# tomtor/HDL-deflate

Hardware: AMD Instinct MI355X
Metric: compress_input_throughput (CWINDOW=32, MATCH10=True, static tree) (higher is better)
Workload: dtype u8; 1 GPU; BASELINE configs[1]: 1048576 x 2048 B blocks, families 1-4 (test_deflate.py:38-66), distinct blocks, HBM-resident; cwindow=32, maxmatch=10, blocks_per_gpu=1048576, block_bytes=2048

## Files before the change

### __graft_entry__.py

```python
import os
import subprocess
import sys

REPO = os.path.dirname(os.path.abspath(__file__))
if REPO not in sys.path:
    sys.path.insert(0, REPO)


def build():
    subprocess.check_call(["bash", os.path.join(REPO, "hdl_deflate_amd", "csrc", "build.sh")])
    subprocess.check_call(["bash", os.path.join(REPO, "hdl_deflate_amd", "csrc", "build.sh"), "forced"])
    subprocess.check_call(["bash", os.path.join(REPO, "hdl_deflate_amd", "csrc", "build.sh"), "keys"])
    subprocess.check_call(["bash", os.path.join(REPO, "hdl_deflate_amd", "csrc", "build.sh"), "alllive"])
    subprocess.check_call(["make", "-s", "-C", os.path.join(REPO, "oracle"), "all"])
    import hdl_deflate_amd
    from hdl_deflate_amd import _lib
    L = _lib.load()
    hdr = open(os.path.join(REPO, "include", "hdlz.h")).read()
    import re
    want = int(re.search(r"#define\s+HDLZ_VERSION\s+(0x[0-9a-fA-F]+)", hdr).group(1), 16)
    assert L.hdlz_version() == want, (hex(L.hdlz_version()), hex(want))
    for name in _lib.EXPORTS:
        assert hasattr(L, name), name
    return None


def smoke():
    import zlib
    import torch
    import hdl_deflate_amd
    from hdl_deflate_amd.data import make_blocks
    from oracle import oracle as O
    assert torch.cuda.is_available(), "smoke() needs cuda:0"
    torch.cuda.set_device(0)
    eng = hdl_deflate_amd.Engine()
    d = make_blocks(64, 2048, "cuda", seed=1)
    out, ol, st = eng.compress_batch(d, cwindow=32, maxmatch=10)
    back, bl, bs = eng.inflate_batch(out, out_pitch=2048)
    torch.cuda.synchronize()
    assert int((st != 0).sum()) == 0 and int((bs != 0).sum()) == 0
    assert torch.equal(back, d)
    h, ho, hl = d.cpu().numpy(), out.cpu().numpy(), ol.cpu().numpy()
    for b in range(64):
        blk = h[b].tobytes()
        z = ho[b, :hl[b]].tobytes()
        rc, ref = O.compress(blk, 32, 10)
        assert rc == 0 and z == ref, "block %d differs from the oracle" % b
        assert zlib.decompress(z) == blk
    blk0 = h[0].tobytes()
    ses = eng.compress_session()
    for k in range(0, len(blk0), 300):
        ses.write(blk0[k:k + 300])
        assert ses.step() == 0
    assert ses.step(final=True) == 0 and ses.done and ses.output(0, ses.out_len) == O.compress(blk0, 32, 10)[1]
    st1, z = eng.compress_bytes(b"Hello World! " * 3)
    assert st1 == 0 and z.hex() == "789cf348cdc9c95708cf2fca4951544070101c10475101000c2f0d18"
    print("smoke OK: 64 x 2 KiB blocks bit-identical to the oracle, zlib round trip, ratio %.3f" %
          (hl.sum() / (64 * 2048.0)))
    return None


if __name__ == "__main__":
    build()
    if len(sys.argv) > 1 and sys.argv[1] == "smoke":
        smoke()
```

### hdl_deflate_amd/csrc/hdlz_compress.hip

```cpp
#include <hip/hip_runtime.h>
#include <stdint.h>
#include "hdlz_device.h"
#include "hdlz_compress_common.h"

namespace hdlz {

#ifndef HDLZ_HP_SEARCH
#define HDLZ_HP_SEARCH 1
#define HDLZ_HP_EXTEND 0
#define HDLZ_HP_REST 0
#endif
#ifdef HDLZ_TILE_TIMING
#define TT_DECL() uint32_t tacc[13] = {0, 0, 0, 0, 0, 0, 0, 0, 0, 0, 0, 0, 0}, tlast = (uint32_t)__builtin_readcyclecounter(); \
        const uint32_t tt_c0 = tlast, tt_r0 = (uint32_t)__builtin_amdgcn_s_memrealtime()
#define TT(k) do { const uint32_t t_ = (uint32_t)__builtin_readcyclecounter(); tacc[k] += t_ - tlast; tlast = t_; } while (0)
#define TT_TILE() tacc[12] += 1u
#else
#define TT_DECL() do {} while (0)
#define TT(k) do {} while (0)
#define TT_TILE() do {} while (0)
#endif

__device__ __forceinline__ void store_words(uint32_t* __restrict__ dst, const uint32_t* lsrc, uint32_t words, uint32_t lane) {
    typedef uint32_t v4 __attribute__((ext_vector_type(4)));
// ... 59 lines not shown
        const uint8_t* t = reinterpret_cast<const uint8_t*>(FIXED_LUT.e) + 16u * lane;
        lds_dma16(t, lut_base);
        lds_dma16(t + 1024u, lut_base + 1024u);
    };

#if defined(HDLZ_STRIDE_PLAIN) || defined(HDLZ_TILE_TIMING)
    constexpr bool MOVING_COLUMN = false;
#else
    constexpr bool MOVING_COLUMN = BITS;
#endif
    [[maybe_unused]] uint64_t row0 = 0;
    [[maybe_unused]] uint32_t col = blockIdx.x;
    auto next_block = [&](uint64_t& blk) {
        if constexpr (MOVING_COLUMN) {
            row0 += gridDim.x;
            col = col + 1u == gridDim.x ? 0u : col + 1u;
            blk = row0 + col;
        } else blk += gridDim.x;
    };
    TT_DECL();
    for (uint64_t blk = blockIdx.x; blk < a.nblocks; next_block(blk)) {
        const uint8_t* src;
        uint32_t n;
        const uint32_t bst = block_params(blk, src, n);
        if (bst != HDLZ_OK) {
            if (lane == 0) {
                a.out_len[blk] = 0; a.status[blk] = bst;
                if constexpr (ENDBITS) a.end_bits[blk] = 0;
            }
            continue;
        }
        uint32_t* __restrict__ outw = reinterpret_cast<uint32_t*>(a.out + blk * a.out_pitch);
        const uint32_t mis = (uint32_t)(reinterpret_cast<uintptr_t>(src) & 3u);
        const bool aligned16 = (reinterpret_cast<uintptr_t>(src) & 15u) == 0;

        uint32_t gw = 0;
        uint32_t base_bits = HEADER_BITS;
        uint32_t carry_word = HEADER_WORD;
        uint32_t skip_in = 0;
        uint32_t ad_a = 0, ad_w = 0;
        uint32_t wm = (n - min(lane * (uint32_t)RUN, n)) % ADLER_MOD;

        for (uint32_t t0 = 0; t0 < n; t0 += TILE) {
            if (blk == blockIdx.x) TT(10); else TT(0);
            HDLZ_MARK("stage");
            const uint32_t nfull = min((n - t0) >> 4, NCHUNK);
            wave_lds_order();
            lds.in[lane] = t0 != 0 ? lds.in[(TILE / 4) + lane] : 0u;
            asm volatile("s_waitcnt lgkmcnt(0)" ::: "memory");
            request_tile(src + t0, nfull);
            {
                const uint32_t part = (nfull < NCHUNK && ((n - t0) & 15u) != 0u) ? 1u : 0u;
                for (uint32_t c = nfull + part + lane; c < NCHUNK; c += 64) *reinterpret_cast<uint4*>(lin8 + HALO + c * 16u) = make_uint4(0, 0, 0, 0);
                if (part) {
                    if (lane == 0u) *reinterpret_cast<uint4*>(lin8 + HALO + nfull * 16u) = load_chunk16(src, t0 + nfull * 16u, n, aligned16, mis);
                }
            }
            if constexpr (!HASH && !BITS) zero_bit_buffer(lout, lane, carry_word);
            asm volatile("s_waitcnt vmcnt(0)" ::: "memory");
            wave_lds_order();

            const uint32_t run_dw = (HALO / 4) + lane * (RUN / 4);
            const uint32_t p_run = t0 + lane * RUN;
            const uint32_t nrem = n - min(p_run, n);
            uint32_t best[RUN], tok[RUN], code[RUN];
            [[maybe_unused]] uint32_t oww[12];
            [[maybe_unused]] bool any = true;
            [[maybe_unused]] uint32_t planes[7];
            if constexpr (BITS) {
                load_own(lds.in, run_dw, oww);
                asm volatile("s_waitcnt lgkmcnt(0)" ::: "memory");
                wave_lds_order();
            }
            TT(1);
            if constexpr (!HASH) __builtin_amdgcn_s_setprio(0);
            else __builtin_amdgcn_s_setprio(HDLZ_HP_SEARCH);
            HDLZ_MARK("search");
            if constexpr (HASH) {
                match_search_hash<NCH>(lds.in, hl, lane, (uint32_t)a.cwindow, best);
                zero_bit_buffer(lout, lane, carry_word);
            }
#ifndef HDLZ_SEARCH_KEYS
            else if constexpr (BITS)
                any = match_search_bits<true>(oww[0], oww[1], oww[2], oww[3], oww[4], oww[5], oww[6], oww[7], planes, lds.neq + lane);
#endif
            else match_search<NCH, ONE_TILE && NCH == 1>(lds.in, run_dw, best);
            {
                TT(2);
                HDLZ_MARK("adler");
                uint32_t ow[12];
                if constexpr (BITS) {
#pragma unroll
                    for (int k = 0; k < 12; k++) ow[k] = oww[k];
                } else load_own(lds.in, run_dw, ow);
                {
                    uint32_t sa, sc;
                    adler_run(ow, sa, sc);
                    ad_a += sa;
                    ad_w = (ad_w + __umul24(wm, sa) + (4u * ADLER_MOD - sc)) % ADLER_MOD;
                    wm = wm >= (uint32_t)(TILE % ADLER_MOD) ? wm - (uint32_t)(TILE % ADLER_MOD) : wm + (ADLER_MOD - (uint32_t)(TILE % ADLER_MOD));
                    if (((t0 >> 11) & 0x3FFFFu) == 0x3FFFFu) ad_a %= ADLER_MOD;
                    asm volatile("" : "+v"(ad_a), "+v"(ad_w), "+v"(wm));
                }
                TT(3);
                if constexpr (!HASH) __builtin_amdgcn_s_setprio(1);
                else __builtin_amdgcn_s_setprio(HDLZ_HP_EXTEND);
                HDLZ_MARK("extend");
                if constexpr (BITS) {
                    if (any) {
                        search_result_bytes(planes, best);
                        wave_lds_order();
                        make_tokens_bits<FULLWIN>(lds.neq, lane, ow, best, cw4, kmax, 4u * min(p_run, 32u * NCH), nrem, tok, (int32_t)(n - t0));
                    } else {
                        literal_tokens(ow, tok);
                        asm volatile("s_waitcnt lgkmcnt(0)" ::: "memory");
                        wave_lds_order();
                    }
                } else
                make_tokens<NCH, FULLWIN, true>(lds.in, HALO + lane * RUN, ow, best, cw4, kmax, 4u * min(p_run, 32u * NCH), nrem, tok, (int32_t)(n - t0));
            }
            pin(tok);
            PHASE_FENCE();
            TT(4);
            if constexpr (BITS) {
                HDLZ_MARK("zero");
                wave_lds_order();
                request_lut();
                zero_bit_buffer(lout, lane, carry_word);
            }
            if constexpr (HASH) __builtin_amdgcn_s_setprio(HDLZ_HP_REST);
            HDLZ_MARK("parse");
            uint32_t myskip = 0;
            if (!BITS || any) {
                const uint64_t P = run_transfer(tok);
                TT(5);
                HDLZ_MARK("chain");
                myskip = chain_skips(P, lane, skip_in);
            }
            pin(tok); asm volatile("" : "+v"(myskip));
            PHASE_FENCE();
            TT(6);
            HDLZ_MARK("codes");
            if constexpr (BITS) {
                asm volatile("s_waitcnt vmcnt(0)" ::: "memory");
                wave_lds_order();
            }
            uint32_t lane_bits = token_codes<NCH, false>(lut8, tok, myskip, 0u, code);
            pin(code);
            PHASE_FENCE();
            TT(7);
            HDLZ_MARK("scan");
            uint32_t incl = wave_scan_incl(lane_bits);
            const uint32_t tile_bits_all = (uint32_t)__builtin_amdgcn_readlane((int)incl, 63);
            pin(code); asm volatile("" : "+v"(incl), "+v"(lane_bits));
            PHASE_FENCE();
            TT(8);
            HDLZ_MARK("scatter");
            scatter_codes(out8, code, base_bits + incl - lane_bits);
            TT(9);
            HDLZ_MARK("flush");
            wave_lds_order();
            TT(10);

            const bool last = ONE_TILE || (t0 + TILE >= n);
            if (!last) {
                const uint32_t end_bits = base_bits + tile_bits_all;
                const uint32_t full = end_bits >> 5;
                store_words(outw + gw, lout, full, lane);
                carry_word = lout[full];
                gw += full;
                base_bits = end_bits & 31u;
            } else {
                const uint32_t ninv = t0 + TILE - n;
                const uint32_t end_bits = base_bits + tile_bits_all - PAD_BITS * ninv;
                if (lane < 4u) wipe_behind(lout, end_bits, lane);
                uint32_t s1, s2;
                adler_finish(wave_sum(ad_a % ADLER_MOD), wave_sum(ad_w), n, s1, s2);
                const uint32_t nbytes = block_nbytes(end_bits);
                wave_lds_order();
                if (lane == 0) put_adler(out8, nbytes, s1, s2);
                wave_lds_order();
                const uint32_t total = nbytes + 4u;
                const uint32_t words = (total + 3u) >> 2;
                store_words(outw + gw, lout, words, lane);
                if (lane == 0) {
                    a.out_len[blk] = gw * 4u + total;
                    a.status[blk] = HDLZ_OK;
                    if constexpr (ENDBITS) a.end_bits[blk] = 32ull * gw + end_bits;
                }
            }
            TT(11);
            TT_TILE();
        }
    }
#ifdef HDLZ_TILE_TIMING
// ... 62 lines not shown
```

### hdl_deflate_amd/csrc/hdlz_compress_common.h

```cpp
#pragma once
#include <hip/hip_runtime.h>
#include <stddef.h>
#include <stdint.h>
#include "hdlz_device.h"
#include "hdlz_adler.h"

namespace hdlz {

#ifndef HDLZ_W1
#define HDLZ_W1 5
#endif

#ifndef HDLZ_EXT_GROUP
#define HDLZ_EXT_GROUP 4
#endif
#ifndef HDLZ_CODE_GROUP
#define HDLZ_CODE_GROUP 4
#endif
constexpr int RUN = 32;
constexpr int TILE = 64 * RUN;
constexpr int HALO = 256;
constexpr int LOOKAHEAD = 16;
constexpr int IN_BYTES = HALO + TILE + LOOKAHEAD;
constexpr int OUT_WORDS = 592;
constexpr int LUT_LIT = 256;
constexpr int LUT_MATCH = 256;
constexpr uint32_t LUT_MATCH_BYTE = 4u * LUT_LIT;
constexpr int LUT_LEN = 16;
constexpr uint32_t LUT_LEN_BYTE = 4u * (LUT_LIT + LUT_MATCH);
constexpr uint32_t NB_SHIFT = 27;
constexpr uint32_t CODE_MASK = (1u << NB_SHIFT) - 1u;

struct __attribute__((aligned(16))) WaveLds {
    uint32_t in[IN_BYTES / 4];
    uint32_t out[OUT_WORDS];
    uint32_t lut[LUT_LIT + LUT_MATCH + LUT_LEN];
};

constexpr uint32_t GATHER_SPAN = 4u * (0x3FFu + 3u);
static_assert(sizeof(WaveLds) >= GATHER_SPAN, "make_tokens: masked gather inside the LDS block");

constexpr int NEQ_ROWS = 32;
constexpr int NEQ_WORDS = NEQ_ROWS * 64;
constexpr int FIXED_LUT_WORDS = LUT_LIT + LUT_MATCH;
constexpr bool search_bits() {
#ifdef HDLZ_SEARCH_KEYS
    return false;
#else
    return true;
#endif
}
struct __attribute__((aligned(16))) WaveLdsBits {
    union {
        uint32_t in[IN_BYTES / 4];
        uint32_t neq[NEQ_WORDS];
        struct {
            uint32_t out[OUT_WORDS];
            uint32_t gap[NEQ_WORDS - OUT_WORDS - FIXED_LUT_WORDS];
            uint32_t lut[FIXED_LUT_WORDS];
        };
    };
};
static_assert((0x7C << 6) + 4 * 63 + 4 <= 4 * NEQ_WORDS && ((0xFF & 0x7C) << 6) == 4 * 64 * 31, "every read of the extension inside NEQ; none -> row 31");
static_assert(((4 * 32) & 0x7C) == 0 && (31 * 64 + 63) < NEQ_WORDS, "d = 32 aliases row 0; the search's last row ends inside NEQ");
static_assert(sizeof(WaveLdsBits) == 8192 && 4 * NEQ_WORDS >= IN_BYTES, "20 waves per CU; the staged tile inside the block");
static_assert(offsetof(WaveLdsBits, lut) >= 4 * OUT_WORDS && offsetof(WaveLdsBits, lut) % 16 == 0 && 4 * FIXED_LUT_WORDS == 2 * 64 * 16,
              "zero_bit_buffer leaves the LUT alone; the LUT is two 16-byte LDS-DMA requests per lane");

struct __attribute__((aligned(16))) WaveLdsNoOut {
    uint32_t in[IN_BYTES / 4];
    uint32_t lut[LUT_LIT + LUT_MATCH + LUT_LEN];
};

#define PHASE_FENCE() __builtin_amdgcn_sched_barrier(0)
#define HDLZ_MARK(name) do { PHASE_FENCE(); asm volatile("; @@PHASE " name ::: "memory"); PHASE_FENCE(); } while (0)
template <int N>
__device__ __forceinline__ void pin(uint32_t (&a)[N]) {
#pragma unroll
    for (int i = 0; i < N; i++) asm volatile("" : "+v"(a[i]));
}
template <int B, int E, int N>
__device__ __forceinline__ void pin_range(uint32_t (&a)[N]) {
#pragma unroll
    for (int i = B; i < E; i++) asm volatile("" : "+v"(a[i]));
}

__device__ __forceinline__ uint32_t alignbyte(uint32_t hi, uint32_t lo, uint32_t sh) {
    return __builtin_amdgcn_alignbyte(hi, lo, sh);
}
__device__ __forceinline__ uint32_t umin3(uint32_t a, uint32_t b, uint32_t c) {
    uint32_t t = a < b ? a : b;
    return t < c ? t : c;
}
__device__ __forceinline__ uint32_t ffbl(uint32_t x) { return (uint32_t)(__builtin_ffs((int)x) - 1); }

template <int J>
__device__ __forceinline__ uint32_t key3(const uint32_t* d, uint32_t tag) {
    constexpr int w = J >> 2, sh = J & 3;
    if constexpr (sh == 0) return (d[w] << 8) | tag;
    else if constexpr (sh == 1) return (d[w] & 0xFFFFFF00u) | tag;
    else return (alignbyte(d[w + 1], d[w], sh - 1) & 0xFFFFFF00u) | tag;
}

__host__ __device__ constexpr uint32_t literal_entry(uint32_t b) {
    const bool big = b >= 144u;
    const uint32_t v = big ? (0x100u + b) : (0x30u + b);
    const uint32_t nb = big ? 9u : 8u;
    return (__builtin_bitreverse32(v) >> (32u - nb)) | (nb << NB_SHIFT);
}
__host__ __device__ constexpr uint32_t dist_entry(uint32_t d) {
    const uint32_t dd = d - 1u;
    uint32_t c = dd, eb = 0, extra = 0;
    if (dd >= 4u) {
        const uint32_t hb = 31u - (uint32_t)__builtin_clz(dd);
        eb = hb - 1u;
        c = 2u * hb + ((dd >> eb) & 1u);
        extra = dd & ((1u << eb) - 1u);
    }
    const uint32_t dcode = __builtin_bitreverse32(c) >> 27;
    return ((dcode | (extra << 5)) << 7) | ((12u + eb) << NB_SHIFT);
}
__host__ __device__ constexpr uint32_t length_code(uint32_t m) { return __builtin_bitreverse32(m - 2u) >> 25; }
static_assert(literal_entry(0) == (0x0Cu | 8u << NB_SHIFT), "literal 0: 8 bits, 00110000 reversed");
static_assert(literal_entry(143) == (0xFDu | 8u << NB_SHIFT), "literal 143: 8 bits, 10111111 reversed");
static_assert(literal_entry(144) == (0x13u | 9u << NB_SHIFT), "literal 144: 9 bits, 110010000 reversed");
static_assert(literal_entry(255) == (0x1FFu | 9u << NB_SHIFT), "literal 255: 9 bits, all ones");
static_assert(length_code(3) == 0x40u && length_code(10) == 0x08u, "lengths 3 / 10: symbols 257 / 264 = 7-bit codes 0000001 / 0001000 reversed");
static_assert(dist_entry(1) == (12u << NB_SHIFT), "distance 1: code 0, no extra bits: 7 + 5 bits");
static_assert(dist_entry(5) == ((0x04u << 7) | 13u << NB_SHIFT), "distance 5: code 4 (00100), one extra bit 0");
static_assert(dist_entry(32) == (((0x12u | 7u << 5) << 7) | 15u << NB_SHIFT), "distance 32: code 9 (01001 reversed), three extra bits 111");

__host__ __device__ constexpr uint32_t match_entry32(uint32_t e) { return dist_entry((e & 31u) + 1u) | length_code((e >> 5) + 3u); }
struct __attribute__((aligned(16))) FixedLut { uint32_t e[LUT_LIT + LUT_MATCH]; };
constexpr FixedLut make_fixed_lut() {
    FixedLut t{};
    for (uint32_t k = 0; k < (uint32_t)LUT_LIT; k++) t.e[k] = literal_entry(k);
    for (uint32_t k = 0; k < (uint32_t)LUT_MATCH; k++) t.e[LUT_LIT + k] = match_entry32(k);
    return t;
}
static __device__ const FixedLut FIXED_LUT = make_fixed_lut();
static_assert(make_fixed_lut().e[LUT_LIT + 32 * 7 + 31] == (dist_entry(32) | length_code(10)), "match [len - 3][dist - 1]");


__device__ __forceinline__ void load_own(const uint32_t* in, uint32_t run_dw, uint32_t (&ow)[12]) {
    const uint4 v0 = *reinterpret_cast<const uint4*>(&in[run_dw]);
    const uint4 v1 = *reinterpret_cast<const uint4*>(&in[run_dw + 4]);
    const uint4 v2 = *reinterpret_cast<const uint4*>(&in[run_dw + 8]);
    ow[0] = v0.x; ow[1] = v0.y; ow[2] = v0.z; ow[3] = v0.w;
// ... 43 lines not shown
                cd[12] = c3.x; cd[13] = c3.y; cd[14] = c3.z; cd[15] = c3.w;
                cd[16] = in[cdw + 16];
            }
        }
        uint32_t m[RUN];
#pragma unroll
        for (int i = 0; i < RUN; i++) m[i] = 0xFFFFFFFFu;
        static_for<0, 63>([&](auto J) {
            constexpr int j = decltype(J)::value;
            if constexpr ((j & 1) == 0) {
                uint32_t kc0, kc1;
                if constexpr (NCH == 1 && j >= 32) {
                    asm volatile("" : "+v"(ko[j - 32]), "+v"(ko[j - 31]));
                    kc0 = ko[j - 32];
                    kc1 = ko[j - 31];
                } else if constexpr (PREV_DPP) {
                    kc0 = (uint32_t)__builtin_amdgcn_update_dpp(0, (int)ko[j], 0x13C, 0xF, 0xF, false) + m128;
                    kc1 = (uint32_t)__builtin_amdgcn_update_dpp(0, (int)ko[j + 1], 0x13C, 0xF, 0xF, false) + m128;
                } else {
                    kc0 = key3<j>(cd, (uint32_t)(4 * j));
                    kc1 = key3<j + 1>(cd, (uint32_t)(4 * (j + 1)));
                }
                static_for<0, RUN>([&](auto I) {
                    constexpr int i = decltype(I)::value;
                    constexpr bool use0 = (j >= i) && (j <= i + 31);
                    constexpr bool use1 = (j + 1 >= i) && (j + 1 <= i + 31);
                    if constexpr (use0 && use1) m[i] = umin3(m[i], ko[i] - kc0, ko[i] - kc1);
                    else if constexpr (use0) m[i] = min(m[i], ko[i] - kc0);
                    else if constexpr (use1) m[i] = min(m[i], ko[i] - kc1);
                });
                if constexpr ((j & 7) == 6) { pin(m); PHASE_FENCE(); }
            }
        });
#pragma unroll
        for (int i = 0; i < RUN; i++) {
            if (NCH == 1) best[i] = m[i];
            else if (m[i] < 256u) best[i] = m[i] + 128u * (uint32_t)k;
        }
    }
}

constexpr uint32_t B3_SEL = 0xE4;
constexpr uint32_t B3_OR_XOR = 0xF6;
constexpr uint32_t B3_OR3 = 0xFE;
constexpr uint32_t B3_OR_ANDN = 0xF4;
template <uint32_t F>
__device__ __forceinline__ uint32_t bitop3(uint32_t a, uint32_t b, uint32_t c) { return __builtin_amdgcn_bitop3_b32(a, b, c, F); }
__device__ __forceinline__ uint32_t sconst(uint32_t v) { asm volatile("" : "+s"(v)); return v; }
__device__ __forceinline__ void exchange8(uint32_t (&w)[8]) {
    static_for<0, 3>([&](auto J) {
        constexpr int s = 1 << decltype(J)::value;
        const uint32_t m0 = sconst(s == 1 ? 0x55555555u : s == 2 ? 0x33333333u : 0x0F0F0F0Fu);
#pragma unroll
        for (int k = 0; k < 8; k++) {
            if (k & s) continue;
            const uint32_t x = w[k], y = w[k + s];
            w[k] = bitop3<B3_SEL>(x, y << s, m0);
            w[k + s] = bitop3<B3_SEL>(x >> s, y, m0);
        }
    });
}
__device__ __forceinline__ void transpose4x4_bytes(uint32_t r0, uint32_t r1, uint32_t r2, uint32_t r3, uint32_t& t0, uint32_t& t1,
                                                   uint32_t& t2, uint32_t& t3) {
    const uint32_t zip_lo = sconst(0x05010400u), zip_hi = sconst(0x07030602u), cat_lo = sconst(0x05040100u), cat_hi = sconst(0x07060302u);
    const uint32_t a01 = __builtin_amdgcn_perm(r1, r0, zip_lo), b01 = __builtin_amdgcn_perm(r1, r0, zip_hi);
    const uint32_t a23 = __builtin_amdgcn_perm(r3, r2, zip_lo), b23 = __builtin_amdgcn_perm(r3, r2, zip_hi);
    t0 = __builtin_amdgcn_perm(a23, a01, cat_lo); t1 = __builtin_amdgcn_perm(a23, a01, cat_hi);
    t2 = __builtin_amdgcn_perm(b23, b01, cat_lo); t3 = __builtin_amdgcn_perm(b23, b01, cat_hi);
}
constexpr bool skip_dead_planes() {
#ifdef HDLZ_PLANES_ALL_LIVE
    return false;
#else
    return true;
#endif
}
constexpr bool literal_tiles() {
#ifdef HDLZ_NO_LITERAL_TILE
    return false;
#else
    return true;
#endif
}
template <bool KEEP>
__device__ __forceinline__ bool match_search_bits(uint32_t x0, uint32_t x1, uint32_t x2, uint32_t x3, uint32_t x4, uint32_t x5, uint32_t x6,
                                                  uint32_t x7, uint32_t (&R)[7], [[maybe_unused]] uint32_t* neq_col = nullptr) {
    uint32_t O[8];
    transpose4x4_bytes(x0, x2, x4, x6, O[0], O[1], O[2], O[3]);
    transpose4x4_bytes(x1, x3, x5, x7, O[4], O[5], O[6], O[7]);
    exchange8(O);
    pin(O);
    PHASE_FENCE();
    uint32_t nq[RUN];
    static_for<0, 8>([&](auto B) {
        constexpr int b = decltype(B)::value;
        bool live = true;
        if constexpr (b != 0 && skip_dead_planes()) {
            const uint32_t s0 = (uint32_t)__builtin_amdgcn_readfirstlane((int)O[b]);
            live = !((s0 == 0u || s0 == 0xFFFFFFFFu) && ballot64(O[b] != s0) == 0ull);
        }
        if (live) {
            const uint32_t Pb = (uint32_t)__builtin_amdgcn_mov_dpp((int)O[b], 0x13C, 0xF, 0xF, false);
            static_for<1, RUN + 1>([&](auto Dd) {
                constexpr int d = decltype(Dd)::value;
                const uint32_t c = d == 32 ? Pb : __builtin_amdgcn_alignbit(O[b], Pb, (uint32_t)(32 - d));
                if constexpr (b == 0) nq[d - 1] = O[0] ^ c;
                else nq[d - 1] = bitop3<B3_OR_XOR>(nq[d - 1], O[b], c);
                if constexpr ((d & 3) == 0) { pin_range<d - 4, d>(nq); PHASE_FENCE(); }
            });
        }
        pin(nq);
        PHASE_FENCE();
    });
    uint32_t G = 0xFFFFFFFFu, D[6] = {0, 0, 0, 0, 0, 0};
    static_for<1, RUN + 1>([&](auto Dd) {
        constexpr int d = decltype(Dd)::value;
        const uint32_t neq = nq[d - 1];
        if constexpr (KEEP) neq_col[(d & (NEQ_ROWS - 1)) * 64] = neq;
        const uint32_t nx = (uint32_t)__builtin_amdgcn_mov_dpp((int)neq, 0x130, 0xF, 0xF, true);
        const uint32_t n3 = bitop3<B3_OR3>(neq, __builtin_amdgcn_alignbit(nx, neq, 1u), __builtin_amdgcn_alignbit(nx, neq, 2u));
        static_for<0, 6>([&](auto K) {
            constexpr int k = decltype(K)::value;
            if constexpr ((d >> k) & 1) D[k] = bitop3<B3_OR_ANDN>(D[k], G, n3);
        });
        G &= n3;
        if constexpr ((d & 3) == 0) { pin(D); asm volatile("" : "+v"(G)); PHASE_FENCE(); }
    });
    R[0] = G;
#pragma unroll
    for (int k = 0; k < 6; k++) R[k + 1] = D[k];
    if constexpr (literal_tiles()) return ballot64(G != 0xFFFFFFFFu) != 0ull;
    else return true;
}
__device__ __forceinline__ void search_result_bytes(const uint32_t (&R)[7], uint32_t (&best)[RUN]) {
    const uint32_t G = R[0];
    uint32_t Q[8] = {G, G, R[1] | G, R[2] | G, R[3] | G, R[4] | G, R[5] | G, R[6] | G};
    exchange8(Q);
#pragma unroll
    for (int k = 0; k < 8; k++) {
        best[k] = Q[k] & 0xFFu;
        best[k + 8] = __builtin_amdgcn_ubfe(Q[k], 8u, 8u);
        best[k + 16] = __builtin_amdgcn_ubfe(Q[k], 16u, 8u);
        best[k + 24] = Q[k] >> 24;
    }
}
template <int NCH> struct HashCfg {
#ifndef HDLZ_HASH_BITS
#define HDLZ_HASH_BITS 10
#endif
    static constexpr int HB = HDLZ_HASH_BITS;
    static constexpr int NT = 1 << HB;
    static constexpr int PRE = 64 * ((32 * NCH + 63) / 64);
    static_assert(PRE <= HALO && HB >= 8 && HB <= 16, "halo / tag position");
    static_assert(32 * NCH <= PRE, "cwindow <= PRE: chain walks must stay inside the entries this tile has written (ADVICE r3)");
};
template <int NCH> struct __attribute__((aligned(16))) HashLds {
    union {
        uint32_t T[HashCfg<NCH>::NT];
        uint16_t D[TILE];
    };
    uint16_t E[HALO + TILE];
    static_assert(sizeof(uint32_t) * HashCfg<NCH>::NT >= sizeof(uint16_t) * TILE, "D overlays T");
};

__device__ __forceinline__ uint32_t* lds_out(WaveLds& l, uint32_t&) { return l.out; }
__device__ __forceinline__ uint32_t* lds_out(WaveLdsBits& l, uint32_t&) { return l.out; }
template <int NCH> __device__ __forceinline__ uint32_t* lds_out(WaveLdsNoOut&, HashLds<NCH>& h) {
    static_assert(sizeof(h.T) >= sizeof(uint32_t) * OUT_WORDS, "the bit buffer overlays T / D");
    return h.T;
}

template <int NCH>
__device__ __forceinline__ void match_search_hash(const uint32_t* in, HashLds<NCH>& hl, uint32_t lane, uint32_t cw, uint32_t (&best)[RUN]) {
    constexpr int HB = HashCfg<NCH>::HB, NT = HashCfg<NCH>::NT, PRE = HashCfg<NCH>::PRE;
    constexpr uint32_t base = HALO - PRE;
    for (uint32_t k = lane * 4u; k < (uint32_t)NT; k += 256u) *reinterpret_cast<uint4*>(&hl.T[k]) = make_uint4(0, 0, 0, 0);
    __syncthreads();

    constexpr int G = 8;
    static_assert(RUN % G == 0 && PRE / 64 <= G, "groups");
    uint32_t res2[RUN / 2];
    struct Grp { uint32_t kw[G], ow[G], c0[G], dd[G]; };
    auto hash_of = [&](uint32_t kw, uint32_t& tag) -> uint32_t {
        uint32_t mix;
        asm("v_mul_u32_u24 %0, %1, %2" : "=v"(mix) : "v"(kw), "v"(0x9E3779u));
        tag = (mix << (HB - 8)) & 0xFF00u;
        return __builtin_amdgcn_ubfe(mix, 24 - HB, HB);
    };
    auto issue = [&](auto G0, auto CNT, Grp& q) {
        constexpr int g0 = decltype(G0)::value, cnt = decltype(CNT)::value;
        uint32_t w0_[cnt], w1_[cnt];
        static_for<0, cnt>([&](auto J) {
            constexpr int j = decltype(J)::value;
            const uint32_t idx = base + 64u * (uint32_t)(g0 + j) + lane;
            w0_[j] = in[idx >> 2]; w1_[j] = in[(idx >> 2) + 1u];
        });
        static_for<0, cnt>([&](auto J) {
            constexpr int j = decltype(J)::value;
            constexpr uint32_t rbase = base + 64u * (uint32_t)(g0 + j);
            q.kw[j] = alignbyte(w1_[j], w0_[j], lane);
            const uint32_t h = hash_of(q.kw[j], q.ow[j]);
            q.c0[j] = __hip_atomic_fetch_max(&hl.T[h], rbase + lane, __ATOMIC_RELAXED, __HIP_MEMORY_SCOPE_WORKGROUP);
        });
    };
    auto reorder = [&](uint32_t rbase, uint32_t kw, uint32_t got) -> uint32_t {
        uint32_t tag;
        const uint32_t h = hash_of(kw, tag);
        uint32_t before = got, nearer = 0u;
        bool has = false;
#pragma unroll 1
        for (uint32_t s_ = 0; s_ < 64u; s_++) {
            const uint32_t hs = (uint32_t)__builtin_amdgcn_readlane((int)h, (int)s_), gs = (uint32_t)__builtin_amdgcn_readlane((int)got, (int)s_);
            if (hs == h) {
                before = min(before, gs);
                if (s_ < lane) { nearer = rbase + s_; has = true; }
            }
        }
        return has ? nearer : before;
    };
    auto consume = [&](auto G0, auto CNT, Grp& q) {
// ... 109 lines not shown
#pragma unroll
    for (int q = 0; q < 8; q++) {
        const uint4 v = *reinterpret_cast<const uint4*>(&D32[dbase + 4u * q]);
        best[4 * q + 0] = __builtin_amdgcn_ubfe(v.x, hsh, 16u); best[4 * q + 1] = __builtin_amdgcn_ubfe(v.y, hsh, 16u);
        best[4 * q + 2] = __builtin_amdgcn_ubfe(v.z, hsh, 16u); best[4 * q + 3] = __builtin_amdgcn_ubfe(v.w, hsh, 16u);
    }
    __syncthreads();
}

#ifndef HDLZ_WH
#define HDLZ_WH 3
#endif
template <int NCH> constexpr bool wide_hash() { return NCH > 1; }
template <int NCH> constexpr int waves_eu() { return NCH == 1 ? HDLZ_W1 : HDLZ_WH; }

template <int NCH, class F> inline void window_case(int cwindow, F& f) {
    static_assert(32 * NCH <= HashCfg<NCH>::PRE && 32 * NCH <= HALO, "the window of this NCH inside what a tile stages and inserts");
    if (cwindow == 32 * NCH) f(std::integral_constant<int, NCH>{}, std::true_type{});
    else f(std::integral_constant<int, NCH>{}, std::false_type{});
}
template <class F> inline void with_window(int cwindow, F&& f) {
    if (cwindow <= 32) window_case<1>(cwindow, f);
    else if (cwindow <= 64) window_case<2>(cwindow, f);
    else window_case<8>(cwindow, f);
}

template <int NCH, bool FULLWIN, bool SCALAR_TAIL = false, uint32_t GMASK = 0x3FFu>
__device__ __forceinline__ void make_tokens(const uint32_t* in, uint32_t lds_run, uint32_t (&ow)[12], uint32_t (&best)[RUN],
                                            uint32_t cw4, uint32_t kmax, uint32_t p4_run, uint32_t nrem, uint32_t (&tok)[RUN],
                                            int32_t tile_rem = 0) {
    pin(best); pin(ow);
    PHASE_FENCE();
    const uint32_t nrem_m5 = nrem - 5u;
    const uint32_t kmax_m3 = kmax - 3u;
    const int32_t rem5 = tile_rem - 5;
    const uint32_t thr = rem5 >= 0 ? ((uint32_t)rem5 & 31u) : 0u;
    const int32_t cnt_hi = rem5 >= 0 ? (rem5 >> 5) + 1 : 0, cnt_lo = rem5 >= 0 ? (rem5 >> 5) : 0;
    const uint64_t m_hi = cnt_hi >= 64 ? ~0ull : ((1ull << cnt_hi) - 1ull), m_lo = cnt_lo >= 64 ? ~0ull : ((1ull << cnt_lo) - 1ull);
    const uint32_t tok_k = (2u << 18) + LUT_MATCH_BYTE - 4u;
    const uint32_t tok_mul = NCH == 1 ? (4u * 65536u + 128u) : 4u * 65536u;
    static_for<0, RUN>([&](auto I) {
        constexpr int i = decltype(I)::value;
        const uint32_t d4 = best[i];
        uint64_t okm = __builtin_amdgcn_ballot_w64(d4 <= p4_run + (uint32_t)(4 * i));
        if constexpr (!FULLWIN) okm &= __builtin_amdgcn_ballot_w64(d4 <= cw4);
        if constexpr (SCALAR_TAIL) okm &= ((uint32_t)i <= thr ? m_hi : m_lo);
        else okm &= __builtin_amdgcn_ballot_w64(nrem >= (uint32_t)(i + 5));
        const uint32_t d = (NCH == 1) ? (d4 >> 2) : __builtin_amdgcn_ubfe(d4, 2u, 9u);
        const uint32_t q = lds_run + (uint32_t)(i + 3) - d;
        const uint32_t qd = (q >> 2) & GMASK;
        const uint32_t a0 = in[qd], a1 = in[qd + 1], a2 = in[qd + 2];
        const uint32_t clo = alignbyte(a1, a0, q), chi = alignbyte(a2, a1, q);
        constexpr int o = i + 3;
        uint32_t olo, ohi;
        if constexpr ((o & 3) == 0) { olo = ow[o >> 2]; ohi = ow[(o >> 2) + 1]; }
        else { olo = alignbyte(ow[(o >> 2) + 1], ow[o >> 2], o & 3); ohi = alignbyte(ow[(o >> 2) + 2], ow[(o >> 2) + 1], o & 3); }
        const uint32_t zhi = ffbl((chi ^ ohi) | 0x80000000u) | 32u;
        uint32_t zlo;
        asm("v_ffbl_b32 %0, %1" : "=v"(zlo) : "v"(clo ^ olo));
        uint32_t zb;
        asm("v_min_u16 %0, %1, %2" : "=v"(zb) : "v"(zlo), "v"(zhi));
        const uint32_t l3 = umin3(zb >> 3, kmax_m3, nrem_m5 - (uint32_t)i);
        constexpr int bsh = 8 * (i & 3);
        uint32_t lit;
        if constexpr (bsh == 0) lit = (ow[i >> 2] << 2) & 0x3FCu;
        else lit = (ow[i >> 2] >> (bsh - 2)) & 0x3FCu;
        uint32_t mt;
        asm("v_mad_u32_u24 %0, %1, %2, %3" : "=v"(mt) : "v"(l3), "s"(tok_mul), "v"(d4 + tok_k));
        asm("v_cndmask_b32_e64 %0, %1, %2, %3" : "=v"(tok[i]) : "v"(lit), "v"(mt), "s"(okm));
        constexpr int EG = HDLZ_EXT_GROUP;
        if constexpr ((i & (EG - 1)) == EG - 1) { pin_range<(i & ~(EG - 1)), (i & ~(EG - 1)) + EG>(tok); PHASE_FENCE(); }
    });
}

template <int I>
__device__ __forceinline__ uint32_t literal_token(const uint32_t (&ow)[12]) {
    constexpr int bsh = 8 * (I & 3);
    if constexpr (bsh == 0) return (ow[I >> 2] << 2) & 0x3FCu;
    else return (ow[I >> 2] >> (bsh - 2)) & 0x3FCu;
}
__device__ __forceinline__ void literal_tokens(const uint32_t (&ow)[12], uint32_t (&tok)[RUN]) {
    static_for<0, RUN>([&](auto I) { tok[decltype(I)::value] = literal_token<decltype(I)::value>(ow); });
}
template <bool FULLWIN>
__device__ __forceinline__ void make_tokens_bits(const uint32_t* neq, uint32_t lane, uint32_t (&ow)[12], uint32_t (&best)[RUN], uint32_t cw4,
                                                 uint32_t kmax, uint32_t p4_run, uint32_t nrem, uint32_t (&tok)[RUN], int32_t tile_rem) {
    pin(best); pin_range<0, 8>(ow);
    PHASE_FENCE();
    const uint32_t nrem_m5 = nrem - 5u;
    const uint32_t kmax_m3 = min(kmax - 3u, 7u);
    const int32_t rem5 = tile_rem - 5;
    const uint32_t thr = rem5 >= 0 ? ((uint32_t)rem5 & 31u) : 0u;
    const int32_t cnt_hi = rem5 >= 0 ? (rem5 >> 5) + 1 : 0, cnt_lo = rem5 >= 0 ? (rem5 >> 5) : 0;
    const uint64_t m_hi = cnt_hi >= 64 ? ~0ull : ((1ull << cnt_hi) - 1ull), m_lo = cnt_lo >= 64 ? ~0ull : ((1ull << cnt_lo) - 1ull);
    const uint32_t tok_k = (2u << 18) + LUT_MATCH_BYTE - 4u;
    const uint32_t tok_mul = 4u * 65536u + 128u;
    const uint8_t* neq8 = reinterpret_cast<const uint8_t*>(neq);
    const uint32_t col_lo = 4u * lane, dcol = 4u * min(lane + 1u, 63u) - col_lo;
    static_for<0, RUN>([&](auto I) {
        constexpr int i = decltype(I)::value;
        const uint32_t d4 = best[i];
        uint64_t okm = __builtin_amdgcn_ballot_w64(d4 <= p4_run + (uint32_t)(4 * i));
        if constexpr (!FULLWIN) okm &= __builtin_amdgcn_ballot_w64(d4 <= cw4);
        okm &= ((uint32_t)i <= thr ? m_hi : m_lo);
        uint32_t a0;
        asm("v_lshl_add_u32 %0, %1, 6, %2" : "=v"(a0) : "v"(d4 & 0x7Cu), "v"(col_lo));
        uint32_t x;
        if constexpr (i + 3 + 7 <= 32) x = *reinterpret_cast<const uint32_t*>(neq8 + a0) >> (i + 3);
        else if constexpr (i + 3 >= 32) x = *reinterpret_cast<const uint32_t*>(neq8 + (a0 + dcol)) >> (i + 3 - 32);
        else x = __builtin_amdgcn_alignbit(*reinterpret_cast<const uint32_t*>(neq8 + (a0 + dcol)), *reinterpret_cast<const uint32_t*>(neq8 + a0), (uint32_t)(i + 3));
        uint32_t z;
        asm("v_ffbl_b32 %0, %1" : "=v"(z) : "v"(x));
        const uint32_t l3 = umin3(z, kmax_m3, nrem_m5 - (uint32_t)i);
        const uint32_t lit = literal_token<i>(ow);
        uint32_t mt;
        asm("v_mad_u32_u24 %0, %1, %2, %3" : "=v"(mt) : "v"(l3), "s"(tok_mul), "v"(d4 + tok_k));
        asm("v_cndmask_b32_e64 %0, %1, %2, %3" : "=v"(tok[i]) : "v"(lit), "v"(mt), "s"(okm));
        constexpr int EG = HDLZ_EXT_GROUP;
        if constexpr ((i & (EG - 1)) == EG - 1) { pin_range<(i & ~(EG - 1)), (i & ~(EG - 1)) + EG>(tok); PHASE_FENCE(); }
    });
}

__device__ __forceinline__ uint64_t run_transfer(const uint32_t (&tok)[RUN]) {
    uint64_t P = 0x9876543210ull;
#pragma unroll
    for (int i = RUN - 1; i >= 0; i--) {
        const uint32_t sh = tok[i] >> 16;
        const uint32_t e = (uint32_t)(P >> sh) & 15u;
        P = (P << 4) | e;
    }
    return P;
}

constexpr int CHAIN_STEPS = 4;
__device__ __forceinline__ uint32_t chain_skips_serial(uint64_t P, uint32_t lane, uint32_t& s);
__device__ __forceinline__ uint32_t chain_skips(uint64_t P, uint32_t lane, uint32_t& s) {
    const uint32_t plo = (uint32_t)P, phi = (uint32_t)(P >> 32) & 0xFFu;
#ifndef HDLZ_CHAIN_SERIAL_ONLY
    const uint32_t dl = plo ^ __builtin_amdgcn_alignbit(phi, plo, 4u), dh = (phi ^ (phi >> 4)) & 15u;
    uint32_t x = (dl | dh) == 0u ? (plo & 15u) : 16u;
#ifdef HDLZ_CHAIN_FORCE_SERIAL
    x = 16u;
#endif
    bool open = ballot64(x >= 16u) != 0ull;
#pragma unroll 1
    for (int it = 0; it < CHAIN_STEPS && open; it++) {
        const uint32_t prev = (uint32_t)__builtin_amdgcn_update_dpp((int)s, (int)x, 0x138, 0xF, 0xF, false);
        const uint32_t via = (uint32_t)(P >> (4u * (prev & 15u))) & 15u;
        x = (x >= 16u && prev < 16u) ? via : x;
        open = ballot64(x >= 16u) != 0ull;
    }
    if (!open) {
        const uint32_t e = (uint32_t)__builtin_amdgcn_update_dpp((int)s, (int)x, 0x138, 0xF, 0xF, false);
        s = (uint32_t)__builtin_amdgcn_readlane((int)x, 63);
        return e;
    }
#endif
    return chain_skips_serial(P, lane, s);
}
__device__ __forceinline__ uint32_t chain_skips_serial(uint64_t P, uint32_t lane, uint32_t& s) {
    const uint32_t plo = (uint32_t)P;
    uint32_t ph4 = (uint32_t)(P >> 32) & 0xFFu;
    ph4 |= (uint32_t)__builtin_amdgcn_mov_dpp((int)ph4, 0xB1, 0xF, 0xF, true) << 8;
    ph4 |= (uint32_t)__builtin_amdgcn_mov_dpp((int)ph4, 0x4E, 0xF, 0xF, true) << 16;
    uint64_t sv[4] = {0, 0, 0, 0};
    static_for<0, 4>([&](auto G) {
        constexpr int g = decltype(G)::value;
        uint64_t acc = 0;
#pragma unroll
        for (int q = 0; q < 4; q++) {
            const uint32_t hi4 = (uint32_t)__builtin_amdgcn_readlane((int)ph4, g * 16 + q * 4);
#pragma unroll
            for (int k = 0; k < 4; k++) {
                const int l = q * 4 + k;
                acc |= (uint64_t)s << (4 * l);
                const uint64_t f = ((uint64_t)((hi4 >> (8 * k)) & 0xFFu) << 32) |
                                   (uint64_t)(uint32_t)__builtin_amdgcn_readlane((int)plo, g * 16 + l);
                s = (uint32_t)(f >> (4u * s)) & 15u;
            }
        }
        sv[g] = acc;
        __builtin_amdgcn_sched_barrier(0);
    });
    const uint32_t g = lane >> 4;
    const uint64_t mine = g == 0 ? sv[0] : g == 1 ? sv[1] : g == 2 ? sv[2] : sv[3];
    return (uint32_t)(mine >> (4u * (lane & 15u))) & 15u;
}

template <int NCH, bool LIMIT>
__device__ __forceinline__ uint32_t token_codes(const uint8_t* lut8, uint32_t (&tok)[RUN], uint32_t c0, uint32_t nlimit,
                                                uint32_t (&code)[RUN]) {
    uint32_t lane_bits = 0;
    uint32_t c = 4u * c0;
    static_for<0, RUN>([&](auto I) {
        constexpr int i = decltype(I)::value;
        const uint32_t e = *reinterpret_cast<const uint32_t*>(lut8 + (tok[i] & 0xFFFFu));
// ... 138 lines not shown
```

Measured before the change: 837,800 MB/s.

## Fold end-of-block cap into search bits and build tokens from packed bytes with SDWA

```diff
diff --git a/__graft_entry__.py b/__graft_entry__.py
--- a/__graft_entry__.py
+++ b/__graft_entry__.py
@@ -12,6 +12,7 @@
     subprocess.check_call(["bash", os.path.join(REPO, "hdl_deflate_amd", "csrc", "build.sh"), "forced"])
     subprocess.check_call(["bash", os.path.join(REPO, "hdl_deflate_amd", "csrc", "build.sh"), "keys"])
     subprocess.check_call(["bash", os.path.join(REPO, "hdl_deflate_amd", "csrc", "build.sh"), "alllive"])
+    subprocess.check_call(["bash", os.path.join(REPO, "hdl_deflate_amd", "csrc", "build.sh"), "dword"])
     subprocess.check_call(["make", "-s", "-C", os.path.join(REPO, "oracle"), "all"])
     import hdl_deflate_amd
     from hdl_deflate_amd import _lib
diff --git a/hdl_deflate_amd/csrc/hdlz_compress.hip b/hdl_deflate_amd/csrc/hdlz_compress.hip
--- a/hdl_deflate_amd/csrc/hdlz_compress.hip
+++ b/hdl_deflate_amd/csrc/hdlz_compress.hip
@@ -165,7 +165,7 @@
             }
 #ifndef HDLZ_SEARCH_KEYS
             else if constexpr (BITS)
-                any = match_search_bits<true>(oww[0], oww[1], oww[2], oww[3], oww[4], oww[5], oww[6], oww[7], planes, lds.neq + lane);
+                any = match_search_bits<true>(oww[0], oww[1], oww[2], oww[3], oww[4], oww[5], oww[6], oww[7], planes, lds.neq + lane, end_cap_word((int32_t)(n - t0) - 2, lane * (uint32_t)RUN));
 #endif
             else match_search<NCH, ONE_TILE && NCH == 1>(lds.in, run_dw, best);
             {
@@ -191,9 +191,16 @@
                 HDLZ_MARK("extend");
                 if constexpr (BITS) {
                     if (any) {
+#if HDLZ_EXT_SDWA
+                        uint32_t Q[8];
+                        search_result_packed(planes, Q);
+                        wave_lds_order();
+                        make_tokens_bits_packed<FULLWIN>(lds.neq, lane, ow, Q, cw4, kmax, tok, (int32_t)(n - t0));
+#else
                         search_result_bytes(planes, best);
                         wave_lds_order();
-                        make_tokens_bits<FULLWIN>(lds.neq, lane, ow, best, cw4, kmax, 4u * min(p_run, 32u * NCH), nrem, tok, (int32_t)(n - t0));
+                        make_tokens_bits<FULLWIN>(lds.neq, lane, ow, best, cw4, kmax, 4u * min(p_run, 32u * NCH), tok, (int32_t)(n - t0));
+#endif
                     } else {
                         literal_tokens(ow, tok);
                         asm volatile("s_waitcnt lgkmcnt(0)" ::: "memory");
diff --git a/hdl_deflate_amd/csrc/hdlz_compress_common.h b/hdl_deflate_amd/csrc/hdlz_compress_common.h
--- a/hdl_deflate_amd/csrc/hdlz_compress_common.h
+++ b/hdl_deflate_amd/csrc/hdlz_compress_common.h
@@ -63,7 +63,7 @@
 };
 static_assert((0x7C << 6) + 4 * 63 + 4 <= 4 * NEQ_WORDS && ((0xFF & 0x7C) << 6) == 4 * 64 * 31, "every read of the extension inside NEQ; none -> row 31");
 static_assert(((4 * 32) & 0x7C) == 0 && (31 * 64 + 63) < NEQ_WORDS, "d = 32 aliases row 0; the search's last row ends inside NEQ");
-static_assert(sizeof(WaveLdsBits) == 8192 && 4 * NEQ_WORDS >= IN_BYTES, "20 waves per CU; the staged tile inside the block");
+static_assert(sizeof(WaveLdsBits) == 8192 && 4 * NEQ_WORDS >= IN_BYTES, "seven allocation steps of 1280 bytes: 18 waves per CU; the staged tile inside the block");
 static_assert(offsetof(WaveLdsBits, lut) >= 4 * OUT_WORDS && offsetof(WaveLdsBits, lut) % 16 == 0 && 4 * FIXED_LUT_WORDS == 2 * 64 * 16,
               "zero_bit_buffer leaves the LUT alone; the LUT is two 16-byte LDS-DMA requests per lane");
 
@@ -273,9 +273,13 @@
     return true;
 #endif
 }
+__device__ __forceinline__ uint32_t end_cap_word(int32_t n_m2, uint32_t p_run) {
+    const int32_t first = min(max(n_m2 - (int32_t)p_run, 0), 32);
+    return (uint32_t)(~0ull << first);
+}
 template <bool KEEP>
 __device__ __forceinline__ bool match_search_bits(uint32_t x0, uint32_t x1, uint32_t x2, uint32_t x3, uint32_t x4, uint32_t x5, uint32_t x6,
-                                                  uint32_t x7, uint32_t (&R)[7], [[maybe_unused]] uint32_t* neq_col = nullptr) {
+                                                  uint32_t x7, uint32_t (&R)[7], [[maybe_unused]] uint32_t* neq_col = nullptr, uint32_t E = 0u) {
     uint32_t O[8];
     transpose4x4_bytes(x0, x2, x4, x6, O[0], O[1], O[2], O[3]);
     transpose4x4_bytes(x1, x3, x5, x7, O[4], O[5], O[6], O[7]);
@@ -295,7 +299,7 @@
             static_for<1, RUN + 1>([&](auto Dd) {
                 constexpr int d = decltype(Dd)::value;
                 const uint32_t c = d == 32 ? Pb : __builtin_amdgcn_alignbit(O[b], Pb, (uint32_t)(32 - d));
-                if constexpr (b == 0) nq[d - 1] = O[0] ^ c;
+                if constexpr (b == 0) nq[d - 1] = bitop3<B3_OR_XOR>(E, O[0], c);
                 else nq[d - 1] = bitop3<B3_OR_XOR>(nq[d - 1], O[b], c);
                 if constexpr ((d & 3) == 0) { pin_range<d - 4, d>(nq); PHASE_FENCE(); }
             });
@@ -323,10 +327,16 @@
     if constexpr (literal_tiles()) return ballot64(G != 0xFFFFFFFFu) != 0ull;
     else return true;
 }
+__device__ __forceinline__ void search_result_packed(const uint32_t (&R)[7], uint32_t (&Q)[8]) {
+    const uint32_t G = R[0];
+    Q[0] = G; Q[1] = G;
+#pragma unroll
+    for (int k = 2; k < 8; k++) Q[k] = R[k - 1] | G;
+    exchange8(Q);
+}
 __device__ __forceinline__ void search_result_bytes(const uint32_t (&R)[7], uint32_t (&best)[RUN]) {
-    const uint32_t G = R[0];
-    uint32_t Q[8] = {G, G, R[1] | G, R[2] | G, R[3] | G, R[4] | G, R[5] | G, R[6] | G};
-    exchange8(Q);
+    uint32_t Q[8];
+    search_result_packed(R, Q);
 #pragma unroll
     for (int k = 0; k < 8; k++) {
         best[k] = Q[k] & 0xFFu;
@@ -602,12 +612,94 @@
 __device__ __forceinline__ void literal_tokens(const uint32_t (&ow)[12], uint32_t (&tok)[RUN]) {
     static_for<0, RUN>([&](auto I) { tok[decltype(I)::value] = literal_token<decltype(I)::value>(ow); });
 }
+#ifndef HDLZ_EXT_SDWA
+#define HDLZ_EXT_SDWA 1
+#endif
+#define HDLZ_SDWA_SRC0_BYTE(op, M) op " %0, %1, %2 dst_sel:DWORD dst_unused:UNUSED_PAD src0_sel:BYTE_" #M " src1_sel:DWORD"
+template <int M> __device__ __forceinline__ uint32_t and_byte(uint32_t q, uint32_t s) {
+    uint32_t r;
+    if constexpr (M == 0) asm(HDLZ_SDWA_SRC0_BYTE("v_and_b32_sdwa", 0) : "=v"(r) : "v"(q), "s"(s));
+    else if constexpr (M == 1) asm(HDLZ_SDWA_SRC0_BYTE("v_and_b32_sdwa", 1) : "=v"(r) : "v"(q), "s"(s));
+    else if constexpr (M == 2) asm(HDLZ_SDWA_SRC0_BYTE("v_and_b32_sdwa", 2) : "=v"(r) : "v"(q), "s"(s));
+    else asm(HDLZ_SDWA_SRC0_BYTE("v_and_b32_sdwa", 3) : "=v"(r) : "v"(q), "s"(s));
+    return r;
+}
+template <int M> __device__ __forceinline__ uint32_t add_byte(uint32_t q, uint32_t s) {
+    uint32_t r;
+    if constexpr (M == 0) asm(HDLZ_SDWA_SRC0_BYTE("v_add_u32_sdwa", 0) : "=v"(r) : "v"(q), "s"(s));
+    else if constexpr (M == 1) asm(HDLZ_SDWA_SRC0_BYTE("v_add_u32_sdwa", 1) : "=v"(r) : "v"(q), "s"(s));
+    else if constexpr (M == 2) asm(HDLZ_SDWA_SRC0_BYTE("v_add_u32_sdwa", 2) : "=v"(r) : "v"(q), "s"(s));
+    else asm(HDLZ_SDWA_SRC0_BYTE("v_add_u32_sdwa", 3) : "=v"(r) : "v"(q), "s"(s));
+    return r;
+}
+#define HDLZ_SDWA_CMP_BYTE(M, S1) "v_cmp_le_u32_sdwa %0, %1, %2 src0_sel:BYTE_" #M " src1_sel:" S1
+template <int M, bool BOTH> __device__ __forceinline__ uint64_t le_byte(uint32_t q, uint32_t s) {
+    uint64_t r;
+    if constexpr (BOTH) {
+        if constexpr (M == 0) asm(HDLZ_SDWA_CMP_BYTE(0, "BYTE_0") : "=s"(r) : "v"(q), "v"(s));
+        else if constexpr (M == 1) asm(HDLZ_SDWA_CMP_BYTE(1, "BYTE_1") : "=s"(r) : "v"(q), "v"(s));
+        else if constexpr (M == 2) asm(HDLZ_SDWA_CMP_BYTE(2, "BYTE_2") : "=s"(r) : "v"(q), "v"(s));
+        else asm(HDLZ_SDWA_CMP_BYTE(3, "BYTE_3") : "=s"(r) : "v"(q), "v"(s));
+    } else {
+        if constexpr (M == 0) asm(HDLZ_SDWA_CMP_BYTE(0, "DWORD") : "=s"(r) : "v"(q), "s"(s));
+        else if constexpr (M == 1) asm(HDLZ_SDWA_CMP_BYTE(1, "DWORD") : "=s"(r) : "v"(q), "s"(s));
+        else if constexpr (M == 2) asm(HDLZ_SDWA_CMP_BYTE(2, "DWORD") : "=s"(r) : "v"(q), "s"(s));
+        else asm(HDLZ_SDWA_CMP_BYTE(3, "DWORD") : "=s"(r) : "v"(q), "s"(s));
+    }
+    return r;
+}
+#define HDLZ_SDWA_SHL_BYTE(M) "v_lshlrev_b32_sdwa %0, %1, %2 dst_sel:DWORD dst_unused:UNUSED_PAD src0_sel:DWORD src1_sel:BYTE_" #M
+template <int M> __device__ __forceinline__ uint32_t shl_byte(uint32_t sh, uint32_t w) {
+    uint32_t r;
+    if constexpr (M == 0) asm(HDLZ_SDWA_SHL_BYTE(0) : "=v"(r) : "s"(sh), "v"(w));
+    else if constexpr (M == 1) asm(HDLZ_SDWA_SHL_BYTE(1) : "=v"(r) : "s"(sh), "v"(w));
+    else if constexpr (M == 2) asm(HDLZ_SDWA_SHL_BYTE(2) : "=v"(r) : "s"(sh), "v"(w));
+    else asm(HDLZ_SDWA_SHL_BYTE(3) : "=v"(r) : "s"(sh), "v"(w));
+    return r;
+}
+template <bool FULLWIN>
+__device__ __forceinline__ void make_tokens_bits_packed(const uint32_t* neq, uint32_t lane, uint32_t (&ow)[12], uint32_t (&Q)[8], uint32_t cw4,
+                                                        uint32_t kmax, uint32_t (&tok)[RUN], int32_t tile_rem) {
+    pin(Q);
+    PHASE_FENCE();
+    const uint32_t kmax_m3 = min(kmax - 3u, 7u);
+    const int32_t rem5 = tile_rem - 5;
+    const uint32_t thr = rem5 >= 0 ? ((uint32_t)rem5 & 31u) : 0u;
+    const int32_t cnt_hi = rem5 >= 0 ? (rem5 >> 5) + 1 : 0, cnt_lo = rem5 >= 0 ? (rem5 >> 5) : 0;
+    const uint64_t m_hi = cnt_hi >= 64 ? ~0ull : ((1ull << cnt_hi) - 1ull), m_lo = cnt_lo >= 64 ? ~0ull : ((1ull << cnt_lo) - 1ull);
+    const uint32_t tok_mul = 4u * 65536u + 128u;
+    const uint8_t* neq8 = reinterpret_cast<const uint8_t*>(neq);
+    const uint32_t col_lo = 4u * lane, dcol = min(252u - col_lo, 4u);
+    const uint32_t tok_k = sconst((2u << 18) + LUT_MATCH_BYTE - 4u), row_mask = sconst(0x7Cu), two = sconst(2u), cw4v = cw4;
+    uint32_t T = lane == 0u ? 0x60402000u : 0xE0C0A080u;
+    asm volatile("" : "+v"(T));
+    static_for<0, RUN>([&](auto J) {
+        constexpr int k = decltype(J)::value >> 2, m = decltype(J)::value & 3, i = k + 8 * m;
+        if constexpr (m == 0 && k != 0) T += 0x04040404u;
+        uint64_t okm = le_byte<m, true>(Q[k], T);
+        if constexpr (!FULLWIN) okm &= le_byte<m, false>(Q[k], cw4v);
+        okm &= ((uint32_t)i <= thr ? m_hi : m_lo);
+        uint32_t a0;
+        asm("v_lshl_add_u32 %0, %1, 6, %2" : "=v"(a0) : "v"(and_byte<m>(Q[k], row_mask)), "v"(col_lo));
+        uint32_t x;
+        if constexpr (i + 3 + 7 <= 32) x = *reinterpret_cast<const uint32_t*>(neq8 + a0) >> (i + 3);
+        else if constexpr (i + 3 >= 32) x = *reinterpret_cast<const uint32_t*>(neq8 + (a0 + dcol)) >> (i + 3 - 32);
+        else x = __builtin_amdgcn_alignbit(*reinterpret_cast<const uint32_t*>(neq8 + (a0 + dcol)), *reinterpret_cast<const uint32_t*>(neq8 + a0), (uint32_t)(i + 3));
+        uint32_t z;
+        asm("v_ffbl_b32 %0, %1" : "=v"(z) : "v"(x));
+        const uint32_t l3 = min(z, kmax_m3);
+        const uint32_t lit = shl_byte<(i & 3)>(two, ow[i >> 2]);
+        uint32_t mt;
+        asm("v_mad_u32_u24 %0, %1, %2, %3" : "=v"(mt) : "v"(l3), "s"(tok_mul), "v"(add_byte<m>(Q[k], tok_k)));
+        asm("v_cndmask_b32_e64 %0, %1, %2, %3" : "=v"(tok[i]) : "v"(lit), "v"(mt), "s"(okm));
+        if constexpr (m == 3) { asm volatile("" : "+v"(tok[k]), "+v"(tok[k + 8]), "+v"(tok[k + 16]), "+v"(tok[k + 24]), "+v"(T)); PHASE_FENCE(); }
+    });
+}
 template <bool FULLWIN>
 __device__ __forceinline__ void make_tokens_bits(const uint32_t* neq, uint32_t lane, uint32_t (&ow)[12], uint32_t (&best)[RUN], uint32_t cw4,
-                                                 uint32_t kmax, uint32_t p4_run, uint32_t nrem, uint32_t (&tok)[RUN], int32_t tile_rem) {
+                                                 uint32_t kmax, uint32_t p4_run, uint32_t (&tok)[RUN], int32_t tile_rem) {
     pin(best); pin_range<0, 8>(ow);
     PHASE_FENCE();
-    const uint32_t nrem_m5 = nrem - 5u;
     const uint32_t kmax_m3 = min(kmax - 3u, 7u);
     const int32_t rem5 = tile_rem - 5;
     const uint32_t thr = rem5 >= 0 ? ((uint32_t)rem5 & 31u) : 0u;
@@ -631,7 +723,7 @@
         else x = __builtin_amdgcn_alignbit(*reinterpret_cast<const uint32_t*>(neq8 + (a0 + dcol)), *reinterpret_cast<const uint32_t*>(neq8 + a0), (uint32_t)(i + 3));
         uint32_t z;
         asm("v_ffbl_b32 %0, %1" : "=v"(z) : "v"(x));
-        const uint32_t l3 = umin3(z, kmax_m3, nrem_m5 - (uint32_t)i);
+        const uint32_t l3 = min(z, kmax_m3);
         const uint32_t lit = literal_token<i>(ow);
         uint32_t mt;
         asm("v_mad_u32_u24 %0, %1, %2, %3" : "=v"(mt) : "v"(l3), "s"(tok_mul), "v"(d4 + tok_k));
```

Measured after the change: 877,000 MB/s, median of 6. +4.7%, better.
